# OpenVisualCloud/SVT-HEVC

Hardware: AMD Instinct MI355X
Metric: front-half fps, 4K 8-bit encMode 7 random-access B pictures (BASELINE configs[2]): pictures per second through upload + picture preparation + open-loop motion estimation of 2040 LCUs against 2 list(s) (HME L0 64x32 + L1, full-pel 16x9 85-PU search, sub-pel, bi-prediction) + open-loop intra search +  (higher is better)
Workload: dtype u8; 1 GPU

## Files before the change

svt-hevc_amd/csrc/prep_kernels.hip:

```cpp
#include "svt_amd_internal.h"

__device__ __forceinline__ int clampi(int v, int lo, int hi) { return v < lo ? lo : (v > hi ? hi : v); }
__device__ __forceinline__ uint32_t round_shift_clip(int sum_plus_16)
{
    const uint32_t u = (uint32_t)(sum_plus_16 < 0 ? 0 : sum_plus_16) >> 5;
    return u > 255u ? 255u : u;
}

#define STRIP 16

struct PrepJobDev {
    const uint8_t *raw;
    int32_t raw_stride, w, h;
    uint8_t *full, *quarter, *sixteenth, *B, *H, *J;
    int32_t pitch_full, pitch_quarter, pitch_sixteenth;
};

__device__ __forceinline__ uint32_t vfilt4(uint32_t m2, uint32_t m1, uint32_t c0, uint32_t p1)
{
    uint32_t v = 0;
#pragma unroll
    for (int i = 0; i < 4; i++) {
        const int s = 8 * i;
        v |= round_shift_clip(-2 * (int)((m2 >> s) & 255) + 18 * (int)((m1 >> s) & 255) + 18 * (int)((c0 >> s) & 255) -
                              2 * (int)((p1 >> s) & 255) + 16) << s;
    }
    return v;
}

__device__ __forceinline__ void load7(const uint8_t *row, int x0, int w, bool fast, int (&a)[7], uint32_t &fd)
{
    if (fast) {
        const uint32_t d0 = *(const uint32_t *)(row + x0 - 4), d1 = *(const uint32_t *)(row + x0),
                       d2 = *(const uint32_t *)(row + x0 + 4);
        a[0] = (d0 >> 16) & 255, a[1] = d0 >> 24;
        a[2] = d1 & 255, a[3] = (d1 >> 8) & 255, a[4] = (d1 >> 16) & 255, a[5] = d1 >> 24;
        a[6] = d2 & 255;
        fd = d1;
    } else {
#pragma unroll
        for (int i = 0; i < 7; i++)
            a[i] = row[clampi(x0 - 2 + i, 0, w - 1)];
        fd = (uint32_t)a[2] | ((uint32_t)a[3] << 8) | ((uint32_t)a[4] << 16) | ((uint32_t)a[5] << 24);
    }
}

__global__ __launch_bounds__(256) void k_prep_fused(const PrepJobDev *__restrict__ jobs, int b0, int b1)
{
    const PrepJobDev J = jobs[blockIdx.y];
    const int w = J.w, h = J.h;
    int blk = (int)blockIdx.x;
    if (blk < b0) {
        const int pad = SVT_AMD_PAD_FULL;
        const int cols4 = (w + 2 * pad) >> 2, strips = (h + 2 * pad + STRIP - 1) / STRIP;
        const int g = blk * 256 + (int)threadIdx.x;
        if (g >= cols4 * strips)
            return;
        const int strip = g / cols4, cx = g - strip * cols4;
        const int x0 = -pad + 4 * cx, ys = -pad + STRIP * strip, ye = min(ys + STRIP, h + pad);
        const bool fast = x0 >= 4 && x0 + 8 <= w && ((((uintptr_t)J.raw) | (uint32_t)J.raw_stride) & 3) == 0;
        uint32_t f[4] = {0, 0, 0, 0}, b[4] = {0, 0, 0, 0};
        const ptrdiff_t pf = J.pitch_full;
        for (int r = ys - 2; r <= ye; r++) {
            const uint8_t *row = J.raw + (size_t)clampi(r, 0, h - 1) * J.raw_stride;
            int a[7];
            uint32_t fd, vb = 0;
            load7(row, x0, w, fast, a, fd);
#pragma unroll
            for (int i = 0; i < 4; i++)
                vb |= round_shift_clip(-2 * a[i] + 18 * a[i + 1] + 18 * a[i + 2] - 2 * a[i + 3] + 16) << (8 * i);
            f[0] = f[1], f[1] = f[2], f[2] = f[3], f[3] = fd;
            b[0] = b[1], b[1] = b[2], b[2] = b[3], b[3] = vb;
            if (r >= ys && r < ye) {
                *(uint32_t *)(J.full + r * pf + x0) = fd;
                *(uint32_t *)(J.B + r * pf + x0) = vb;
            }
            const int y = r - 1;
            if (y >= ys && y < ye && r >= ys + 1) {
                *(uint32_t *)(J.H + y * pf + x0) = vfilt4(f[0], f[1], f[2], f[3]);
                *(uint32_t *)(J.J + y * pf + x0) = vfilt4(b[0], b[1], b[2], b[3]);
            }
        }
        return;
    }
    const bool q = blk < b0 + b1;
    blk -= q ? b0 : b0 + b1;
    const int step = q ? 2 : 4, pad = q ? SVT_AMD_PAD_QUARTER : SVT_AMD_PAD_SIXTEENTH;
    const int dw = w / step, dh = h / step;
    uint8_t *dst = q ? J.quarter : J.sixteenth;
    const ptrdiff_t pitch = q ? J.pitch_quarter : J.pitch_sixteenth;
    const int cols4 = (dw + 2 * pad + 3) >> 2, strips = (dh + 2 * pad + 7) / 8;
    const int g = blk * 256 + (int)threadIdx.x;
    if (g >= cols4 * strips)
        return;
    const int strip = g / cols4, cx = g - strip * cols4;
    const int x0 = -pad + 4 * cx, ys = -pad + 8 * strip, ye = min(ys + 8, dh + pad);
    const bool fast = x0 >= 0 && x0 + 4 <= dw && ((((uintptr_t)J.raw) | (uint32_t)J.raw_stride) & (q ? 7 : 15)) == 0;
    for (int y = ys; y < ye; y++) {
        const uint8_t *row = J.raw + (size_t)(clampi(y, 0, dh - 1) * step) * J.raw_stride;
        uint32_t v;
        if (fast && q) {
            const uint2 d = *(const uint2 *)(row + x0 * 2);
            v = __builtin_amdgcn_perm(d.y, d.x, 0x06040200u);
        } else if (fast) {
            const uint4 d = *(const uint4 *)(row + x0 * 4);
            v = (d.x & 255) | ((d.y & 255) << 8) | ((d.z & 255) << 16) | ((d.w & 255) << 24);
        } else {
            v = 0;
#pragma unroll
            for (int i = 0; i < 4; i++)
                v |= (uint32_t)row[clampi(x0 + i, 0, dw - 1) * step] << (8 * i);
        }
        *(uint32_t *)(dst + y * pitch + x0) = v;
    }
}

static_assert(sizeof(PrepJobDev) <= 128, "context.hip reserves 128 bytes per prep descriptor");

int svt_amd_launch_prep_batch(SvtAmdContext *ctx, DevPicture *const *pics, const uint8_t *const *d_luma, uint32_t stride,
                              int n)
{
    static thread_local PrepJobDev host[SVT_AMD_MAX_BATCH];
    const int w = pics[0]->width, h = pics[0]->height;
    for (int i = 0; i < n; i++) {
        const DevPicture *p = pics[i];
        PrepJobDev &j = host[i];
        j.raw = d_luma[i], j.raw_stride = (int)stride, j.w = w, j.h = h;
        j.full = p->full.origin, j.quarter = p->quarter.origin, j.sixteenth = p->sixteenth.origin;
        j.B = p->hp_b.origin, j.H = p->hp_h.origin, j.J = p->hp_j.origin;
        j.pitch_full = p->full.pitch, j.pitch_quarter = p->quarter.pitch, j.pitch_sixteenth = p->sixteenth.pitch;
    }
    const int padf = SVT_AMD_PAD_FULL;
    const int n0 = ((w + 2 * padf) >> 2) * ((h + 2 * padf + STRIP - 1) / STRIP);
    const int n1 = (((w >> 1) + 2 * SVT_AMD_PAD_QUARTER + 3) >> 2) * (((h >> 1) + 2 * SVT_AMD_PAD_QUARTER + 7) / 8);
    const int n2 = (((w >> 2) + 2 * SVT_AMD_PAD_SIXTEENTH + 3) >> 2) * (((h >> 2) + 2 * SVT_AMD_PAD_SIXTEENTH + 7) / 8);
    const int b0 = (n0 + 255) / 256, b1 = (n1 + 255) / 256, b2 = (n2 + 255) / 256;
    int rc = svt_amd_stamp_begin(ctx, KC_PREP);
    if (rc)
        return rc;
    {
        const int rcd = svt_amd_upload_descriptors(ctx, ctx->d_prep_jobs, host, sizeof(PrepJobDev) * (size_t)n);
        if (rcd)
            return rcd;
    }
    hipLaunchKernelGGL(k_prep_fused, dim3(b0 + b1 + b2, n), dim3(256), 0, svt_amd_ctx_stream(ctx), (const PrepJobDev *)ctx->d_prep_jobs, b0, b1);
    HIP_TRY(hipGetLastError());
    return svt_amd_stamp_end(ctx);
}

int svt_amd_launch_prep(SvtAmdContext *ctx, DevPicture *pic, const uint8_t *d_luma, uint32_t stride)
{
    return svt_amd_launch_prep_batch(ctx, &pic, &d_luma, stride, 1);
}
```

Before: 4773 fps.

## Widen prep full-res lanes to 16 columns with packed 16-bit half-pel filters

Each full-resolution prep thread now covers 16 columns instead of 4, using 128-bit loads and stores. The half-pel filter is computed on even/odd byte halves as packed u16x2 saturating arithmetic, which reduces per-pixel ALU work. Interior lanes are grouped so that the aligned fast path runs in uniform wavefronts. The block size drops to 128 with a waves-per-EU hint, and rows are software-pipelined by loading two rows ahead. Trade-offs are more registers per thread and fewer threads, plus a shared host/device header that adds complexity.

```diff
diff --git a/svt-hevc_amd/csrc/prep_kernels.hip b/svt-hevc_amd/csrc/prep_kernels.hip
--- a/svt-hevc_amd/csrc/prep_kernels.hip
+++ b/svt-hevc_amd/csrc/prep_kernels.hip
@@ -1,118 +1,28 @@
 #include "svt_amd_internal.h"
 
-__device__ __forceinline__ int clampi(int v, int lo, int hi) { return v < lo ? lo : (v > hi ? hi : v); }
-__device__ __forceinline__ uint32_t round_shift_clip(int sum_plus_16)
-{
-    const uint32_t u = (uint32_t)(sum_plus_16 < 0 ? 0 : sum_plus_16) >> 5;
-    return u > 255u ? 255u : u;
-}
+#define PREP_FN static __host__ __device__ __forceinline__
+#include "prep_logic.h"
 
-#define STRIP 16
+static_assert(PREP_PAD == SVT_AMD_PAD_FULL && PREP_PAD_QUARTER == SVT_AMD_PAD_QUARTER && PREP_PAD_SIXTEENTH == SVT_AMD_PAD_SIXTEENTH, "prep_logic.h restates the pads");
 
-struct PrepJobDev {
-    const uint8_t *raw;
-    int32_t raw_stride, w, h;
-    uint8_t *full, *quarter, *sixteenth, *B, *H, *J;
-    int32_t pitch_full, pitch_quarter, pitch_sixteenth;
-};
+typedef PrepJob PrepJobDev;
 
-__device__ __forceinline__ uint32_t vfilt4(uint32_t m2, uint32_t m1, uint32_t c0, uint32_t p1)
-{
-    uint32_t v = 0;
-#pragma unroll
-    for (int i = 0; i < 4; i++) {
-        const int s = 8 * i;
-        v |= round_shift_clip(-2 * (int)((m2 >> s) & 255) + 18 * (int)((m1 >> s) & 255) + 18 * (int)((c0 >> s) & 255) -
-                              2 * (int)((p1 >> s) & 255) + 16) << s;
-    }
-    return v;
-}
-
-__device__ __forceinline__ void load7(const uint8_t *row, int x0, int w, bool fast, int (&a)[7], uint32_t &fd)
-{
-    if (fast) {
-        const uint32_t d0 = *(const uint32_t *)(row + x0 - 4), d1 = *(const uint32_t *)(row + x0),
-                       d2 = *(const uint32_t *)(row + x0 + 4);
-        a[0] = (d0 >> 16) & 255, a[1] = d0 >> 24;
-        a[2] = d1 & 255, a[3] = (d1 >> 8) & 255, a[4] = (d1 >> 16) & 255, a[5] = d1 >> 24;
-        a[6] = d2 & 255;
-        fd = d1;
-    } else {
-#pragma unroll
-        for (int i = 0; i < 7; i++)
-            a[i] = row[clampi(x0 - 2 + i, 0, w - 1)];
-        fd = (uint32_t)a[2] | ((uint32_t)a[3] << 8) | ((uint32_t)a[4] << 16) | ((uint32_t)a[5] << 24);
-    }
-}
-
-__global__ __launch_bounds__(256) void k_prep_fused(const PrepJobDev *__restrict__ jobs, int b0, int b1)
+__global__ __launch_bounds__(PREP_BLOCK) __attribute__((amdgpu_waves_per_eu(4))) void k_prep_fused(const PrepJobDev *__restrict__ jobs, int b0, int b1)
 {
     const PrepJobDev J = jobs[blockIdx.y];
-    const int w = J.w, h = J.h;
+    const PrepGrid G = prep_grid(J.w, J.h);
     int blk = (int)blockIdx.x;
     if (blk < b0) {
-        const int pad = SVT_AMD_PAD_FULL;
-        const int cols4 = (w + 2 * pad) >> 2, strips = (h + 2 * pad + STRIP - 1) / STRIP;
-        const int g = blk * 256 + (int)threadIdx.x;
-        if (g >= cols4 * strips)
-            return;
-        const int strip = g / cols4, cx = g - strip * cols4;
-        const int x0 = -pad + 4 * cx, ys = -pad + STRIP * strip, ye = min(ys + STRIP, h + pad);
-        const bool fast = x0 >= 4 && x0 + 8 <= w && ((((uintptr_t)J.raw) | (uint32_t)J.raw_stride) & 3) == 0;
-        uint32_t f[4] = {0, 0, 0, 0}, b[4] = {0, 0, 0, 0};
-        const ptrdiff_t pf = J.pitch_full;
-        for (int r = ys - 2; r <= ye; r++) {
-            const uint8_t *row = J.raw + (size_t)clampi(r, 0, h - 1) * J.raw_stride;
-            int a[7];
-            uint32_t fd, vb = 0;
-            load7(row, x0, w, fast, a, fd);
-#pragma unroll
-            for (int i = 0; i < 4; i++)
-                vb |= round_shift_clip(-2 * a[i] + 18 * a[i + 1] + 18 * a[i + 2] - 2 * a[i + 3] + 16) << (8 * i);
-            f[0] = f[1], f[1] = f[2], f[2] = f[3], f[3] = fd;
-            b[0] = b[1], b[1] = b[2], b[2] = b[3], b[3] = vb;
-            if (r >= ys && r < ye) {
-                *(uint32_t *)(J.full + r * pf + x0) = fd;
-                *(uint32_t *)(J.B + r * pf + x0) = vb;
-            }
-            const int y = r - 1;
-            if (y >= ys && y < ye && r >= ys + 1) {
-                *(uint32_t *)(J.H + y * pf + x0) = vfilt4(f[0], f[1], f[2], f[3]);
-                *(uint32_t *)(J.J + y * pf + x0) = vfilt4(b[0], b[1], b[2], b[3]);
-            }
-        }
+        const int g = blk * PREP_BLOCK + (int)threadIdx.x;
+        if (g < G.n0)
+            prep_full_lane(&J, &G, g);
         return;
     }
     const bool q = blk < b0 + b1;
     blk -= q ? b0 : b0 + b1;
-    const int step = q ? 2 : 4, pad = q ? SVT_AMD_PAD_QUARTER : SVT_AMD_PAD_SIXTEENTH;
-    const int dw = w / step, dh = h / step;
-    uint8_t *dst = q ? J.quarter : J.sixteenth;
-    const ptrdiff_t pitch = q ? J.pitch_quarter : J.pitch_sixteenth;
-    const int cols4 = (dw + 2 * pad + 3) >> 2, strips = (dh + 2 * pad + 7) / 8;
-    const int g = blk * 256 + (int)threadIdx.x;
-    if (g >= cols4 * strips)
-        return;
-    const int strip = g / cols4, cx = g - strip * cols4;
-    const int x0 = -pad + 4 * cx, ys = -pad + 8 * strip, ye = min(ys + 8, dh + pad);
-    const bool fast = x0 >= 0 && x0 + 4 <= dw && ((((uintptr_t)J.raw) | (uint32_t)J.raw_stride) & (q ? 7 : 15)) == 0;
-    for (int y = ys; y < ye; y++) {
-        const uint8_t *row = J.raw + (size_t)(clampi(y, 0, dh - 1) * step) * J.raw_stride;
-        uint32_t v;
-        if (fast && q) {
-            const uint2 d = *(const uint2 *)(row + x0 * 2);
-            v = __builtin_amdgcn_perm(d.y, d.x, 0x06040200u);
-        } else if (fast) {
-            const uint4 d = *(const uint4 *)(row + x0 * 4);
-            v = (d.x & 255) | ((d.y & 255) << 8) | ((d.z & 255) << 16) | ((d.w & 255) << 24);
-        } else {
-            v = 0;
-#pragma unroll
-            for (int i = 0; i < 4; i++)
-                v |= (uint32_t)row[clampi(x0 + i, 0, dw - 1) * step] << (8 * i);
-        }
-        *(uint32_t *)(dst + y * pitch + x0) = v;
-    }
+    const int g = blk * PREP_BLOCK + (int)threadIdx.x;
+    if (g < (q ? G.n1 : G.n2))
+        prep_decimated_lane(&J, q, g);
 }
 
 static_assert(sizeof(PrepJobDev) <= 128, "context.hip reserves 128 bytes per prep descriptor");
@@ -130,11 +40,8 @@
         j.B = p->hp_b.origin, j.H = p->hp_h.origin, j.J = p->hp_j.origin;
         j.pitch_full = p->full.pitch, j.pitch_quarter = p->quarter.pitch, j.pitch_sixteenth = p->sixteenth.pitch;
     }
-    const int padf = SVT_AMD_PAD_FULL;
-    const int n0 = ((w + 2 * padf) >> 2) * ((h + 2 * padf + STRIP - 1) / STRIP);
-    const int n1 = (((w >> 1) + 2 * SVT_AMD_PAD_QUARTER + 3) >> 2) * (((h >> 1) + 2 * SVT_AMD_PAD_QUARTER + 7) / 8);
-    const int n2 = (((w >> 2) + 2 * SVT_AMD_PAD_SIXTEENTH + 3) >> 2) * (((h >> 2) + 2 * SVT_AMD_PAD_SIXTEENTH + 7) / 8);
-    const int b0 = (n0 + 255) / 256, b1 = (n1 + 255) / 256, b2 = (n2 + 255) / 256;
+    const PrepGrid G = prep_grid(w, h);
+    const int b0 = (G.n0 + PREP_BLOCK - 1) / PREP_BLOCK, b1 = (G.n1 + PREP_BLOCK - 1) / PREP_BLOCK, b2 = (G.n2 + PREP_BLOCK - 1) / PREP_BLOCK;
     int rc = svt_amd_stamp_begin(ctx, KC_PREP);
     if (rc)
         return rc;
@@ -143,7 +50,7 @@
         if (rcd)
             return rcd;
     }
-    hipLaunchKernelGGL(k_prep_fused, dim3(b0 + b1 + b2, n), dim3(256), 0, svt_amd_ctx_stream(ctx), (const PrepJobDev *)ctx->d_prep_jobs, b0, b1);
+    hipLaunchKernelGGL(k_prep_fused, dim3(b0 + b1 + b2, n), dim3(PREP_BLOCK), 0, svt_amd_ctx_stream(ctx), (const PrepJobDev *)ctx->d_prep_jobs, b0, b1);
     HIP_TRY(hipGetLastError());
     return svt_amd_stamp_end(ctx);
 }
diff --git a/svt-hevc_amd/csrc/prep_logic.h b/svt-hevc_amd/csrc/prep_logic.h
--- /dev/null
+++ b/svt-hevc_amd/csrc/prep_logic.h
@@ -0,0 +1,256 @@
+#ifndef SVT_AMD_PREP_LOGIC_H
+#define SVT_AMD_PREP_LOGIC_H
+#include <stddef.h>
+#include <stdint.h>
+
+#ifndef PREP_FN
+#define PREP_FN static inline
+#endif
+#ifndef PREP_STRIP
+#define PREP_STRIP 16
+#endif
+#ifndef PREP_BLOCK
+#define PREP_BLOCK 128
+#endif
+#if defined(__HIP_DEVICE_COMPILE__)
+#define PREP_MEM __attribute__((address_space(1)))
+#else
+#define PREP_MEM
+#endif
+#define PREP_PAD 68
+#define PREP_PAD_QUARTER 32
+#define PREP_PAD_SIXTEENTH 16
+#define PREP_GRID_LEFT 80
+#define PREP_LEFT_ITEMS 6
+
+typedef struct PrepJob {
+    const uint8_t *raw;
+    int32_t raw_stride, w, h;
+    uint8_t *full, *quarter, *sixteenth, *B, *H, *J;
+    int32_t pitch_full, pitch_quarter, pitch_sixteenth;
+} PrepJob;
+
+typedef struct PrepGrid {
+    int32_t interior;
+    int32_t others;
+    int32_t strips;
+    int32_t n0, n1, n2;
+} PrepGrid;
+
+typedef uint32_t prep_u32x2 __attribute__((ext_vector_type(2)));
+typedef uint32_t prep_u32x4 __attribute__((ext_vector_type(4)));
+typedef uint16_t prep_u16x2 __attribute__((ext_vector_type(2)));
+
+PREP_FN int prep_clamp(int v, int lo, int hi) { return v < lo ? lo : (v > hi ? hi : v); }
+
+PREP_FN PrepGrid prep_grid(int w, int h)
+{
+    PrepGrid G;
+    const int items = (((w + PREP_PAD + 15) & ~15) + PREP_GRID_LEFT) / 16;
+    G.interior = (w - 20) / 16;
+    G.others = items - G.interior;
+    G.strips = (h + 2 * PREP_PAD + PREP_STRIP - 1) / PREP_STRIP;
+    G.n0 = items * G.strips;
+    G.n1 = (((w >> 1) + 2 * PREP_PAD_QUARTER + 3) >> 2) * (((h >> 1) + 2 * PREP_PAD_QUARTER + 7) / 8);
+    G.n2 = (((w >> 2) + 2 * PREP_PAD_SIXTEENTH + 3) >> 2) * (((h >> 2) + 2 * PREP_PAD_SIXTEENTH + 7) / 8);
+    return G;
+}
+
+
+PREP_FN uint32_t prep_even(uint32_t d) { return d & 0x00ff00ffu; }
+PREP_FN uint32_t prep_odd(uint32_t d)
+{
+#if defined(__HIP_DEVICE_COMPILE__)
+    return __builtin_amdgcn_perm(0u, d, 0x0c030c01u);
+#else
+    return (d >> 8) & 0x00ff00ffu;
+#endif
+}
+PREP_FN uint32_t prep_between(uint32_t lo, uint32_t hi) { return (lo >> 16) | (hi << 16); }
+PREP_FN uint32_t prep_pack(uint32_t even, uint32_t odd) { return even | (odd << 8); }
+
+PREP_FN uint32_t prep_filt(uint32_t m2, uint32_t m1, uint32_t c0, uint32_t p1)
+{
+    const prep_u16x2 k9 = {9, 9}, k8 = {8, 8}, k4 = {4, 4}, k255 = {255, 255};
+    const prep_u16x2 inner = __builtin_bit_cast(prep_u16x2, m1) + __builtin_bit_cast(prep_u16x2, c0);
+    const prep_u16x2 outer = __builtin_bit_cast(prep_u16x2, m2) + __builtin_bit_cast(prep_u16x2, p1);
+    const prep_u16x2 k = __builtin_elementwise_sub_sat(inner * k9 + k8, outer);
+    return __builtin_bit_cast(uint32_t, __builtin_elementwise_min(k >> k4, k255));
+}
+
+typedef struct PrepRaw { uint32_t d[6]; } PrepRaw;
+typedef struct PrepHalves { uint32_t e[4], o[4]; } PrepHalves;
+
+typedef struct PrepLane {
+    int32_t x0, ys, ye;
+    uint32_t mask;
+    int32_t wide;
+} PrepLane;
+
+
+PREP_FN PrepRaw prep_load_row(const PrepJob *J, const PrepLane *L, int r, int fast)
+{
+    const uint8_t *row = J->raw + (size_t)prep_clamp(r, 0, J->h - 1) * J->raw_stride;
+    PrepRaw R;
+    if (fast) {
+        const uint8_t *p = row + L->x0;
+        R.d[0] = *(const PREP_MEM uint32_t *)(p - 4);
+        if (L->wide) {
+            const prep_u32x4 v = *(const PREP_MEM prep_u32x4 *)p;
+            R.d[1] = v.x, R.d[2] = v.y, R.d[3] = v.z, R.d[4] = v.w;
+        } else {
+            for (int k = 0; k < 4; k++)
+                R.d[1 + k] = *(const PREP_MEM uint32_t *)(p + 4 * k);
+        }
+        R.d[5] = *(const PREP_MEM uint32_t *)(p + 16);
+    } else {
+        for (int k = 0; k < 6; k++) {
+            uint32_t v = 0;
+            for (int i = k ? 0 : 2; i < (k < 5 ? 4 : 1); i++)
+                v |= (uint32_t)((const PREP_MEM uint8_t *)row)[prep_clamp(L->x0 - 4 + 4 * k + i, 0, J->w - 1)] << (8 * i);
+            R.d[k] = v;
+        }
+    }
+    return R;
+}
+
+PREP_FN void prep_store_item(uint8_t *p, uint32_t a, uint32_t b, uint32_t c, uint32_t d, uint32_t mask)
+{
+    if (mask == 15u) {
+        const prep_u32x4 v = {a, b, c, d};
+        *(PREP_MEM prep_u32x4 *)p = v;
+    } else {
+        if (mask & 1u) *(PREP_MEM uint32_t *)p = a;
+        if (mask & 2u) *(PREP_MEM uint32_t *)(p + 4) = b;
+        if (mask & 4u) *(PREP_MEM uint32_t *)(p + 8) = c;
+        if (mask & 8u) *(PREP_MEM uint32_t *)(p + 12) = d;
+    }
+}
+
+PREP_FN void prep_row_step(const PrepJob *J, const PrepLane *L, int r, const PrepRaw *R, const PrepHalves *F0, const PrepHalves *F1, const PrepHalves *F2,
+                           PrepHalves *F3, const PrepHalves *B0, const PrepHalves *B1, const PrepHalves *B2, PrepHalves *B3, int fast)
+{
+    const uint32_t mask = fast ? 15u : L->mask;
+    uint32_t e[6], o[5];
+    for (int k = 0; k < 6; k++)
+        e[k] = prep_even(R->d[k]);
+    for (int k = 0; k < 5; k++)
+        o[k] = prep_odd(R->d[k]);
+    for (int k = 0; k < 4; k++) {
+        const uint32_t eL = prep_between(e[k], e[k + 1]);
+        const uint32_t oL = prep_between(o[k], o[k + 1]);
+        const uint32_t eR = prep_between(e[k + 1], e[k + 2]);
+        F3->e[k] = e[k + 1], F3->o[k] = o[k + 1];
+        B3->e[k] = prep_filt(eL, oL, e[k + 1], o[k + 1]);
+        B3->o[k] = prep_filt(oL, e[k + 1], o[k + 1], eR);
+    }
+    const size_t pitch = (size_t)J->pitch_full, corner = (size_t)PREP_PAD * pitch + PREP_GRID_LEFT;
+    const uint32_t col = (uint32_t)(L->x0 + PREP_GRID_LEFT);
+    if (r >= L->ys && r < L->ye) {
+        const size_t at = (size_t)(uint32_t)(r + PREP_PAD) * pitch + col;
+        prep_store_item(J->full - corner + at, R->d[1], R->d[2], R->d[3], R->d[4], mask);
+        prep_store_item(J->B - corner + at, prep_pack(B3->e[0], B3->o[0]), prep_pack(B3->e[1], B3->o[1]), prep_pack(B3->e[2], B3->o[2]),
+                        prep_pack(B3->e[3], B3->o[3]), mask);
+    }
+    const int y = r - 1;
+    if (y >= L->ys && y < L->ye) {
+        uint32_t hv[4], jv[4];
+        for (int k = 0; k < 4; k++) {
+            hv[k] = prep_pack(prep_filt(F0->e[k], F1->e[k], F2->e[k], F3->e[k]), prep_filt(F0->o[k], F1->o[k], F2->o[k], F3->o[k]));
+            jv[k] = prep_pack(prep_filt(B0->e[k], B1->e[k], B2->e[k], B3->e[k]), prep_filt(B0->o[k], B1->o[k], B2->o[k], B3->o[k]));
+        }
+        const size_t at = (size_t)(uint32_t)(y + PREP_PAD) * pitch + col;
+        prep_store_item(J->H - corner + at, hv[0], hv[1], hv[2], hv[3], mask);
+        prep_store_item(J->J - corner + at, jv[0], jv[1], jv[2], jv[3], mask);
+    }
+}
+
+PREP_FN void prep_strip(const PrepJob *J, PrepLane *L, int fast)
+{
+    if (!fast) {
+        L->mask = 0;
+        for (int k = 0; k < 4; k++)
+            if (L->x0 + 4 * k >= -PREP_PAD && L->x0 + 4 * k + 4 <= J->w + PREP_PAD)
+                L->mask |= 1u << k;
+    }
+    PrepHalves F[4], B[4];
+    for (int i = 0; i < 4; i++)
+        for (int k = 0; k < 4; k++)
+            F[i].e[k] = F[i].o[k] = B[i].e[k] = B[i].o[k] = 0;
+    PrepRaw cur = prep_load_row(J, L, L->ys - 2, fast), next = prep_load_row(J, L, L->ys - 1, fast), ahead = next;
+    for (int r = L->ys - 2; r <= L->ye; r += 4) {
+#if defined(__clang__)
+#pragma unroll
+#endif
+        for (int i = 0; i < 4; i++) {
+            if (fast)
+                ahead = prep_load_row(J, L, r + i + 2, fast);
+            else if (i || r > L->ys - 2)
+                cur = prep_load_row(J, L, r + i, fast);
+            prep_row_step(J, L, r + i, &cur, &F[(i + 1) & 3], &F[(i + 2) & 3], &F[(i + 3) & 3], &F[i], &B[(i + 1) & 3], &B[(i + 2) & 3], &B[(i + 3) & 3], &B[i], fast);
+            if (fast)
+                cur = next, next = ahead;
+        }
+    }
+}
+
+PREP_FN void prep_full_lane(const PrepJob *J, const PrepGrid *G, int g)
+{
+    const int first_other = G->interior * G->strips;
+    PrepLane L;
+    int strip, item, interior = g < first_other;
+    if (interior) {
+        strip = g / G->interior;
+        item = PREP_LEFT_ITEMS + (g - strip * G->interior);
+    } else {
+        const int n = g - first_other;
+        strip = n / G->others;
+        item = n - strip * G->others;
+        if (item >= PREP_LEFT_ITEMS)
+            item += G->interior;
+    }
+    const uintptr_t align = (uintptr_t)J->raw | (uint32_t)J->raw_stride;
+    L.x0 = -PREP_GRID_LEFT + 16 * item;
+    L.ys = -PREP_PAD + PREP_STRIP * strip;
+    L.ye = L.ys + PREP_STRIP < J->h + PREP_PAD ? L.ys + PREP_STRIP : J->h + PREP_PAD;
+    L.wide = (align & 15) == 0;
+    L.mask = 15u;
+    if (interior && (align & 3) == 0)
+        prep_strip(J, &L, 1);
+    else
+        prep_strip(J, &L, 0);
+}
+
+PREP_FN void prep_decimated_lane(const PrepJob *J, int quarter, int g)
+{
+    const int step = quarter ? 2 : 4, pad = quarter ? PREP_PAD_QUARTER : PREP_PAD_SIXTEENTH;
+    const int dw = J->w / step, dh = J->h / step;
+    uint8_t *dst = quarter ? J->quarter : J->sixteenth;
+    const ptrdiff_t pitch = quarter ? J->pitch_quarter : J->pitch_sixteenth;
+    const int cols4 = (dw + 2 * pad + 3) >> 2;
+    const int strip = g / cols4, cx = g - strip * cols4;
+    const int x0 = -pad + 4 * cx, ys = -pad + 8 * strip, ye = ys + 8 < dh + pad ? ys + 8 : dh + pad;
+    const int fast = x0 >= 0 && x0 + 4 <= dw && ((((uintptr_t)J->raw) | (uint32_t)J->raw_stride) & (quarter ? 7 : 15)) == 0;
+    for (int y = ys; y < ye; y++) {
+        const uint8_t *row = J->raw + (size_t)(prep_clamp(y, 0, dh - 1) * step) * J->raw_stride;
+        uint32_t v;
+        if (fast && quarter) {
+            const prep_u32x2 d = *(const PREP_MEM prep_u32x2 *)(row + x0 * 2);
+#if defined(__HIP_DEVICE_COMPILE__)
+            v = __builtin_amdgcn_perm(d.y, d.x, 0x06040200u);
+#else
+            v = (d.x & 255u) | ((d.x >> 8) & 0xff00u) | ((d.y & 255u) << 16) | ((d.y << 8) & 0xff000000u);
+#endif
+        } else if (fast) {
+            const prep_u32x4 d = *(const PREP_MEM prep_u32x4 *)(row + x0 * 4);
+            v = (d.x & 255u) | ((d.y & 255u) << 8) | ((d.z & 255u) << 16) | ((d.w & 255u) << 24);
+        } else {
+            v = 0;
+            for (int i = 0; i < 4; i++)
+                v |= (uint32_t)((const PREP_MEM uint8_t *)row)[prep_clamp(x0 + i, 0, dw - 1) * step] << (8 * i);
+        }
+        *(PREP_MEM uint32_t *)(dst + y * pitch + x0) = v;
+    }
+}
+
+#endif
```

Result: slower. 4719 fps (-1.1%).
